# yisol/IDM-VTON

Hardware: NVIDIA H100
Metric: try-on images/sec @768x1024, 30 steps, CFG 2.0 (higher is better)
Workload: dtype fp16

## Files before the change

idm-vton_b200/csrc/attn.cu:

```cuda
#include "common.cuh"
#include "host.h"
#include "wgmma.cuh"

namespace vton {

struct FlashParams {
  __half* out;
  int ld_out;
  int B, H, Nq, N0, N1;
  int D;
  int kv1_off;
  int kv1_count;
  const int* kv1_base;
  int causal;
  float scale_log2;
  int accumulate;
  float out_scale;
};

constexpr int FA_REGION = 128 * 128;
constexpr int FA_STAGES = 2;
constexpr int FA_THREADS = 256;

template <int R>
struct FlashSmem {
  static constexpr int OFF_Q = 0;
  static constexpr int OFF_K = OFF_Q + R * FA_REGION;
  static constexpr int OFF_V = OFF_K + FA_STAGES * R * FA_REGION;
  static constexpr int OFF_BAR = OFF_V + FA_STAGES * R * FA_REGION;
  static constexpr int TOTAL = OFF_BAR + 64 + 1024;
};

__device__ __forceinline__ float fast_exp2(float x) {
  float y;
  asm("ex2.approx.ftz.f32 %0, %1;" : "=f"(y) : "f"(x));
  return y;
}

template <int KS, int R = (KS + 3) / 4, int DN = (KS <= 4 ? 64 : 96)>
__global__ void __launch_bounds__(FA_THREADS, 1)
flash_kernel(const __grid_constant__ CUtensorMap tmQ, const __grid_constant__ CUtensorMap tmK0,
             const __grid_constant__ CUtensorMap tmV0, const __grid_constant__ CUtensorMap tmK1,
             const __grid_constant__ CUtensorMap tmV1, const FlashParams p) {
  using SM = FlashSmem<R>;
  extern __shared__ uint8_t smem_raw[];
  const uint32_t smem_base = (smem_u32(smem_raw) + 1023u) & ~1023u;
  const uint32_t bar_base = smem_base + SM::OFF_BAR;
  const uint32_t q_full = bar_base;
  auto kv_full = [&](int s) { return bar_base + 8u * (1 + s); };
  auto kv_empty = [&](int s) { return bar_base + 8u * (1 + FA_STAGES + s); };

  const int warp = threadIdx.x >> 5;
  const int lane = threadIdx.x & 31;
  const int q_tile = blockIdx.x;
  const int h = blockIdx.y;
  const int b = blockIdx.z;

  if (threadIdx.x == 0) {
    tma_prefetch_desc(&tmQ);
    tma_prefetch_desc(&tmK0);
    tma_prefetch_desc(&tmV0);
    if (p.N1 > 0) {
      tma_prefetch_desc(&tmK1);
      tma_prefetch_desc(&tmV1);
    }
    mbar_init(q_full, 1);
    for (int s = 0; s < FA_STAGES; ++s) {
      mbar_init(kv_full(s), 1);
      mbar_init(kv_empty(s), 2);
    }
    fence_barrier_init();
  }
  pdl_wait();
  __syncthreads();
  pdl_launch_dependents();

  const int tiles0 = (p.N0 + 127) >> 7;
  int idx1 = -1;
  if (p.N1 > 0) {
    idx1 = b - p.kv1_off;
    if (idx1 >= 0) idx1 = idx1 % p.kv1_count + (p.kv1_base ? *p.kv1_base : 0);
  }
  const bool zero_kv = (p.N1 > 0) && (idx1 < 0);
  const int tiles1 = (p.N1 > 0 && idx1 >= 0) ? ((p.N1 + 127) >> 7) : 0;
  const int total = p.causal ? min(tiles0, q_tile + 1) : tiles0 + tiles1;

  auto issue_kv = [&](int j) {
    const int stage = j % FA_STAGES;
    if (j >= FA_STAGES) mbar_wait(kv_empty(stage), ((j / FA_STAGES) - 1) & 1);
    mbar_expect_tx(kv_full(stage), 2 * R * FA_REGION);
#pragma unroll
    for (int r = 0; r < R; ++r) {
      const uint32_t kdst = smem_base + SM::OFF_K + (stage * R + r) * FA_REGION;
      const uint32_t vdst = smem_base + SM::OFF_V + (stage * R + r) * FA_REGION;
      const int col = h * p.D + r * 64;
      if (j < tiles0) {
        tma_load_3d(kdst, &tmK0, kv_full(stage), col, j * 128, b);
        tma_load_3d(vdst, &tmV0, kv_full(stage), col, j * 128, b);
      } else {
        tma_load_3d(kdst, &tmK1, kv_full(stage), col, (j - tiles0) * 128, idx1);
        tma_load_3d(vdst, &tmV1, kv_full(stage), col, (j - tiles0) * 128, idx1);
      }
    }
  };
  if (threadIdx.x == 0) {
    mbar_expect_tx(q_full, R * FA_REGION);
#pragma unroll
    for (int r = 0; r < R; ++r)
      tma_load_3d(smem_base + SM::OFF_Q + r * FA_REGION, &tmQ, q_full, h * p.D + r * 64, q_tile * 128, b);
    for (int j = 0; j < FA_STAGES && j < total; ++j) issue_kv(j);
  }

  const int wg = warp >> 2;
  const int row0 = wg * 64 + ((warp & 3) << 4) + (lane >> 2);
  const int qi0 = q_tile * 128 + row0, qi1 = qi0 + 8;
  const int cq = (lane & 3) * 2;
  const float sl2 = p.scale_log2;
  float m0 = -INFINITY, m1 = -INFINITY, l0 = 0.f, l1 = 0.f;
  float o[DN / 2];
#pragma unroll
  for (int i = 0; i < DN / 2; ++i) o[i] = 0.f;

  mbar_wait(q_full, 0);
  const uint32_t q_src = smem_base + SM::OFF_Q + wg * (64 * 128);
  for (int j = 0; j < total; ++j) {
    const int stage = j % FA_STAGES;
    mbar_wait(kv_full(stage), (j / FA_STAGES) & 1);
    const uint32_t k_src = smem_base + SM::OFF_K + stage * R * FA_REGION;
    const uint32_t v_src = smem_base + SM::OFF_V + stage * R * FA_REGION;
    float s[64];
    wgmma_fence();
#pragma unroll
    for (int k = 0; k < KS; ++k) {
      const uint32_t off = (k >> 2) * FA_REGION + (k & 3) * 32;
      WgmmaF16SS<128, 0>::mma(s, make_gmma_desc_sw128(q_src + off, 0, 1024), make_gmma_desc_sw128(k_src + off, 0, 1024),
                              k > 0 ? 1 : 0);
    }
    wgmma_commit();
    wgmma_wait<0>();
    fence_regs(s);

    const int key0 = (j < tiles0) ? j * 128 : (j - tiles0) * 128;
    const int kv_valid = (j < tiles0) ? min(128, p.N0 - key0) : min(128, p.N1 - key0);
    float mx0 = -INFINITY, mx1 = -INFINITY;
#pragma unroll
    for (int i = 0; i < 16; ++i) {
#pragma unroll
      for (int u = 0; u < 2; ++u) {
        const int col = i * 8 + cq + u;
        bool ok = col < kv_valid;
        const bool ok0 = ok && (!p.causal || key0 + col <= qi0);
        const bool ok1 = ok && (!p.causal || key0 + col <= qi1);
        if (!ok0) s[4 * i + u] = -INFINITY;
        if (!ok1) s[4 * i + 2 + u] = -INFINITY;
        mx0 = fmaxf(mx0, s[4 * i + u]);
        mx1 = fmaxf(mx1, s[4 * i + 2 + u]);
      }
    }
    mx0 = fmaxf(mx0, __shfl_xor_sync(0xffffffffu, mx0, 1));
    mx0 = fmaxf(mx0, __shfl_xor_sync(0xffffffffu, mx0, 2));
    mx1 = fmaxf(mx1, __shfl_xor_sync(0xffffffffu, mx1, 1));
    mx1 = fmaxf(mx1, __shfl_xor_sync(0xffffffffu, mx1, 2));
    const float mn0 = fmaxf(m0, mx0), mn1 = fmaxf(m1, mx1);
    const float alpha0 = fast_exp2((m0 - mn0) * sl2), alpha1 = fast_exp2((m1 - mn1) * sl2);
    const float ms0 = mn0 * sl2, ms1 = mn1 * sl2;
    m0 = mn0;
    m1 = mn1;
    float sum0 = 0.f, sum1 = 0.f;
#pragma unroll
    for (int i = 0; i < 16; ++i) {
#pragma unroll
      for (int u = 0; u < 2; ++u) {
        const float x0 = s[4 * i + u], x1 = s[4 * i + 2 + u];
        const float p0 = x0 == -INFINITY ? 0.f : fast_exp2(x0 * sl2 - ms0);
        const float p1 = x1 == -INFINITY ? 0.f : fast_exp2(x1 * sl2 - ms1);
        s[4 * i + u] = p0;
        s[4 * i + 2 + u] = p1;
        sum0 += p0;
        sum1 += p1;
      }
    }
    l0 = l0 * alpha0 + sum0;
    l1 = l1 * alpha1 + sum1;
#pragma unroll
    for (int i = 0; i < DN / 8; ++i) {
      o[4 * i] *= alpha0;
      o[4 * i + 1] *= alpha0;
      o[4 * i + 2] *= alpha1;
      o[4 * i + 3] *= alpha1;
    }
    uint32_t pa[8][4];
#pragma unroll
    for (int kk = 0; kk < 8; ++kk) {
      pa[kk][0] = pack_h2(s[8 * kk + 0], s[8 * kk + 1]);
      pa[kk][1] = pack_h2(s[8 * kk + 2], s[8 * kk + 3]);
      pa[kk][2] = pack_h2(s[8 * kk + 4], s[8 * kk + 5]);
      pa[kk][3] = pack_h2(s[8 * kk + 6], s[8 * kk + 7]);
    }
    fence_regs(o);
    wgmma_fence();
#pragma unroll
    for (int kk = 0; kk < 8; ++kk)
      WgmmaF16RS<DN>::mma(o, pa[kk], make_gmma_desc_sw128(v_src + kk * 2048, FA_REGION, 1024), 1);
    wgmma_commit();
    wgmma_wait<0>();
    fence_regs(o);
    if ((threadIdx.x & 127) == 0) mbar_arrive(kv_empty(stage));
    if (threadIdx.x == 0 && j + FA_STAGES < total) issue_kv(j + FA_STAGES);
  }

  l0 += __shfl_xor_sync(0xffffffffu, l0, 1);
  l0 += __shfl_xor_sync(0xffffffffu, l0, 2);
  l1 += __shfl_xor_sync(0xffffffffu, l1, 1);
  l1 += __shfl_xor_sync(0xffffffffu, l1, 2);
  if (zero_kv) {
    const float mn0 = fmaxf(m0, 0.f), mn1 = fmaxf(m1, 0.f);
    const float alpha0 = fast_exp2((m0 - mn0) * sl2), alpha1 = fast_exp2((m1 - mn1) * sl2);
    l0 = l0 * alpha0 + static_cast<float>(p.N1) * fast_exp2(-mn0 * sl2);
    l1 = l1 * alpha1 + static_cast<float>(p.N1) * fast_exp2(-mn1 * sl2);
#pragma unroll
    for (int i = 0; i < DN / 8; ++i) {
      o[4 * i] *= alpha0;
      o[4 * i + 1] *= alpha0;
      o[4 * i + 2] *= alpha1;
      o[4 * i + 3] *= alpha1;
    }
  }
  const float inv[2] = {1.f / l0, 1.f / l1};
  const int qi[2] = {qi0, qi1};
#pragma unroll
  for (int hr = 0; hr < 2; ++hr) {
    if (qi[hr] >= p.Nq) continue;
    __half* dst = p.out + (static_cast<long long>(b) * p.Nq + qi[hr]) * p.ld_out + h * p.D;
#pragma unroll
    for (int i = 0; i < DN / 8; ++i) {
      const int col = i * 8 + cq;
      if (col >= p.D) continue;
      float v0 = o[4 * i + 2 * hr] * inv[hr], v1 = o[4 * i + 2 * hr + 1] * inv[hr];
      if (p.accumulate) {
        const float2 a = unpack_h2(*reinterpret_cast<const uint32_t*>(dst + col));
        v0 = a.x + round_h(p.out_scale * round_h(v0));
        v1 = a.y + round_h(p.out_scale * round_h(v1));
      }
      *reinterpret_cast<uint32_t*>(dst + col) = pack_h2(v0, v1);
    }
  }
}

void set_attn_poly(int) {}
void set_attn_qtiles(int) {}
void set_attn_v2(int) {}

static int encode_tokens(CUtensorMap* tm, const void* base, long long ld, int cols, int n, int batch) {
  uint64_t dims[3] = {static_cast<uint64_t>(cols), static_cast<uint64_t>(n), static_cast<uint64_t>(batch)};
  uint64_t strides[2] = {static_cast<uint64_t>(ld) * 2, static_cast<uint64_t>(n) * ld * 2};
  uint32_t box[3] = {64, 128, 1};
  return encode_tmap_f16(tm, base, 3, dims, strides, box);
}

template <int KS>
static int launch_flash(const CUtensorMap& tmQ, const CUtensorMap& tmK0, const CUtensorMap& tmV0, const CUtensorMap& tmK1,
                        const CUtensorMap& tmV1, const FlashParams& p, cudaStream_t stream) {
  constexpr int R = (KS + 3) / 4;
  auto kern = flash_kernel<KS>;
  static bool configured = false;
  if (!configured) {
    VTON_CUDA(cudaFuncSetAttribute(kern, cudaFuncAttributeMaxDynamicSharedMemorySize, FlashSmem<R>::TOTAL));
    configured = true;
  }
  dim3 grid((p.Nq + 127) / 128, p.H, p.B);
  VTON_CUDA(launch_kernel(kern, grid, dim3(FA_THREADS), FlashSmem<R>::TOTAL, stream, tmQ, tmK0, tmV0, tmK1, tmV1, p));
  count_launch();
  return kOk;
}

static int flash(const void* q, long long ldq, const void* k0, const void* v0, long long ldkv0, const void* k1,
                 const void* v1, long long ldkv1, int B1, void* out, long long ldo, FlashParams p, cudaStream_t stream) {
  CUtensorMap tmQ, tmK0, tmV0, tmK1, tmV1;
  const int cols = p.H * p.D;
  if (int e = encode_tokens(&tmQ, q, ldq, cols, p.Nq, p.B)) return e;
  if (int e = encode_tokens(&tmK0, k0, ldkv0, cols, p.N0, p.B)) return e;
  if (int e = encode_tokens(&tmV0, v0, ldkv0, cols, p.N0, p.B)) return e;
  tmK1 = tmK0;
  tmV1 = tmV0;
  if (k1 != nullptr) {
    if (int e = encode_tokens(&tmK1, k1, ldkv1, cols, p.N1, B1)) return e;
    if (int e = encode_tokens(&tmV1, v1, ldkv1, cols, p.N1, B1)) return e;
  }
  p.out = static_cast<__half*>(out);
  p.ld_out = static_cast<int>(ldo);
  switch (p.D / 16) {
    case 1: return launch_flash<1>(tmQ, tmK0, tmV0, tmK1, tmV1, p, stream);
    case 2: return launch_flash<2>(tmQ, tmK0, tmV0, tmK1, tmV1, p, stream);
    case 3: return launch_flash<3>(tmQ, tmK0, tmV0, tmK1, tmV1, p, stream);
    case 4: return launch_flash<4>(tmQ, tmK0, tmV0, tmK1, tmV1, p, stream);
    case 5: return launch_flash<5>(tmQ, tmK0, tmV0, tmK1, tmV1, p, stream);
    case 6: return launch_flash<6>(tmQ, tmK0, tmV0, tmK1, tmV1, p, stream);
  }
  set_last_error("attention: head dim %d unsupported", p.D);
  return kErrUnsupported;
}

int attn_impl(const void* q, long long ldq, const void* k0, const void* v0, long long ldkv0, const void* k1,
              const void* v1, long long ldkv1, void* out, long long ldo, int B, int H, int Nq, int N0, int N1, int B1,
              int kv1_off, int kv1_mod, const void* kv1_base, float scale, int accumulate, cudaStream_t stream) {
  VTON_CHECK_ARG(B > 0 && H > 0 && Nq > 0 && N0 > 0 && N1 >= 0, "attn: bad sizes B=%d H=%d Nq=%d N0=%d N1=%d", B, H, Nq, N0, N1);
  VTON_CHECK_ARG(ldq % 8 == 0 && ldkv0 % 8 == 0 && ldo % 8 == 0, "attn: row strides must be multiples of 8");
  VTON_CHECK_ARG(aligned_to(out, 4), "attn: out must be 4-byte aligned (stored two halves at a time)");
  VTON_CHECK_ARG(B <= 65535 && H <= 65535, "attn: grid too large");
  const bool has1 = N1 > 0 && B1 > 0 && k1 && v1;
  VTON_CHECK_ARG(N1 == 0 || has1 || kv1_off >= B, "attn: segment 1 declared (N1=%d) but no K/V given", N1);
  VTON_CHECK_ARG(!has1 || ldkv1 % 8 == 0, "attn: ldkv1 must be a multiple of 8");
  FlashParams p{};
  p.B = B;
  p.H = H;
  p.Nq = Nq;
  p.N0 = N0;
  p.N1 = N1;
  p.D = 64;
  p.kv1_off = has1 ? kv1_off : (N1 > 0 ? B : 0);
  p.kv1_count = has1 ? (kv1_mod > 0 ? kv1_mod : B1) : 1;
  p.kv1_base = has1 ? static_cast<const int*>(kv1_base) : nullptr;
  p.scale_log2 = scale * 1.4426950408889634f;
  p.accumulate = accumulate;
  p.out_scale = 1.f;
  return flash(q, ldq, k0, v0, ldkv0, has1 ? k1 : nullptr, has1 ? v1 : nullptr, ldkv1, B1, out, ldo, p, stream);
}

int cross_attn_impl(const void* q, long long ldq, const void* kt, const void* vt, long long ldkv_t, int Nt,
                    const void* ki, const void* vi, long long ldkv_i, int Ni, void* out, long long ldo, int B, int H,
                    int Nq, float scale, float ip_scale, cudaStream_t stream) {
  VTON_CHECK_ARG(B > 0 && H > 0 && Nq > 0, "cross_attn: bad sizes B=%d H=%d Nq=%d", B, H, Nq);
  VTON_CHECK_ARG(Nt > 0 && Nt <= 80 && Ni >= 0 && Ni <= 16, "cross_attn: needs 1 <= Nt <= 80 and Ni <= 16 (got %d, %d)", Nt, Ni);
  VTON_CHECK_ARG(q && kt && vt && out && (Ni == 0 || (ki && vi)), "cross_attn: null pointer");
  VTON_CHECK_ARG(ldq % 8 == 0 && ldkv_t % 8 == 0 && ldo % 8 == 0 && (Ni == 0 || ldkv_i % 8 == 0),
                 "cross_attn: row strides must be multiples of 8");
  VTON_CHECK_ARG(aligned_to(out, 4), "cross_attn: out must be 4-byte aligned (stored two halves at a time)");
  VTON_CHECK_ARG(B <= 65535 && H <= 65535, "cross_attn: grid too large");
  FlashParams p{};
  p.B = B;
  p.H = H;
  p.Nq = Nq;
  p.N0 = Nt;
  p.D = 64;
  p.kv1_count = 1;
  p.scale_log2 = scale * 1.4426950408889634f;
  p.out_scale = 1.f;
  if (int e = flash(q, ldq, kt, vt, ldkv_t, nullptr, nullptr, 0, 0, out, ldo, p, stream)) return e;
  if (Ni == 0) return kOk;
  p.N0 = Ni;
  p.accumulate = 1;
  p.out_scale = ip_scale;
  return flash(q, ldq, ki, vi, ldkv_i, nullptr, nullptr, 0, 0, out, ldo, p, stream);
}

int enc_attn_impl(const void* q, long long ldq, const void* k, const void* v, long long ldkv, void* out, long long ldo,
                  int B, int H, int N, int D, float scale, int causal, cudaStream_t stream) {
  VTON_CHECK_ARG(B > 0 && H > 0 && N > 0, "encoder_attention: bad sizes B=%d H=%d N=%d", B, H, N);
  VTON_CHECK_ARG(D >= 16 && D <= 96 && D % 16 == 0, "encoder_attention: head dim %d unsupported (16..96, multiple of 16)", D);
  VTON_CHECK_ARG(ldq % 8 == 0 && ldkv % 8 == 0 && ldo % 8 == 0, "encoder_attention: row strides must be multiples of 8");
  VTON_CHECK_ARG(aligned_to(out, 4), "encoder_attention: out must be 4-byte aligned (stored two halves at a time)");
  VTON_CHECK_ARG(B <= 65535 && H <= 65535, "encoder_attention: grid too large");
  FlashParams p{};
  p.B = B;
  p.H = H;
  p.Nq = N;
  p.N0 = N;
  p.D = D;
  p.kv1_count = 1;
  p.causal = causal ? 1 : 0;
  p.scale_log2 = scale * 1.4426950408889634f;
  p.out_scale = 1.f;
  return flash(q, ldq, k, v, ldkv, nullptr, nullptr, 0, 0, out, ldo, p, stream);
}

}
```

idm-vton_b200/csrc/common.cuh:

```cuda
#pragma once
#include <cuda.h>
#include <cuda_fp16.h>
#include <cuda_runtime.h>
#include <stdint.h>
#include <stdio.h>

namespace vton {


__device__ __forceinline__ uint32_t smem_u32(const void* p) {
  return static_cast<uint32_t>(__cvta_generic_to_shared(p));
}

__device__ __forceinline__ uint64_t globaltimer_ns() {
  uint64_t t;
  asm volatile("mov.u64 %0, %globaltimer;" : "=l"(t));
  return t;
}

__device__ __forceinline__ void mbar_init(uint32_t bar, uint32_t count) {
  asm volatile("mbarrier.init.shared::cta.b64 [%0], %1;" ::"r"(bar), "r"(count) : "memory");
}
__device__ __forceinline__ void fence_barrier_init() {
  asm volatile("fence.mbarrier_init.release.cluster;" ::: "memory");
}
__device__ __forceinline__ void mbar_expect_tx(uint32_t bar, uint32_t bytes) {
  asm volatile("mbarrier.arrive.expect_tx.shared::cta.b64 _, [%0], %1;" ::"r"(bar), "r"(bytes) : "memory");
}
__device__ __forceinline__ void mbar_arrive(uint32_t bar) {
  asm volatile("mbarrier.arrive.shared::cta.b64 _, [%0];" ::"r"(bar) : "memory");
}
__device__ __forceinline__ bool mbar_try_wait(uint32_t bar, uint32_t parity) {
  uint32_t ok;
  asm volatile(
      "{\n\t.reg .pred p;\n\t"
      "mbarrier.try_wait.parity.shared::cta.b64 p, [%1], %2;\n\t"
      "selp.u32 %0, 1, 0, p;\n\t}"
      : "=r"(ok)
      : "r"(bar), "r"(parity)
      : "memory");
  return ok != 0;
}
__device__ __forceinline__ void mbar_wait(uint32_t bar, uint32_t parity) {
  if (mbar_try_wait(bar, parity)) return;
  const uint64_t t0 = globaltimer_ns();
  uint32_t spins = 0;
  while (!mbar_try_wait(bar, parity)) {
    if ((++spins & 0x3ff) == 0 && globaltimer_ns() - t0 > 4000000000ull) __trap();
  }
}

__device__ __forceinline__ void fence_proxy_async_smem() {
  asm volatile("fence.proxy.async.shared::cta;" ::: "memory");
}

__device__ __forceinline__ bool elect_one() {
  uint32_t pred;
  asm volatile(
      "{\n\t.reg .pred p;\n\t"
      "elect.sync _|p, 0xffffffff;\n\t"
      "selp.u32 %0, 1, 0, p;\n\t}"
      : "=r"(pred));
  return pred != 0;
}

__device__ __forceinline__ void tma_prefetch_desc(const CUtensorMap* m) {
  asm volatile("prefetch.tensormap [%0];" ::"l"(reinterpret_cast<uint64_t>(m)) : "memory");
}
__device__ __forceinline__ void tma_load_2d(uint32_t dst, const CUtensorMap* m, uint32_t bar, int c0, int c1) {
  asm volatile(
      "cp.async.bulk.tensor.2d.shared::cluster.global.mbarrier::complete_tx::bytes [%0], [%1, {%3, %4}], [%2];"
      ::"r"(dst), "l"(reinterpret_cast<uint64_t>(m)), "r"(bar), "r"(c0), "r"(c1)
      : "memory");
}
__device__ __forceinline__ void tma_load_3d(uint32_t dst, const CUtensorMap* m, uint32_t bar, int c0, int c1,
                                            int c2) {
  asm volatile(
      "cp.async.bulk.tensor.3d.shared::cluster.global.mbarrier::complete_tx::bytes [%0], [%1, {%3, %4, %5}], [%2];"
      ::"r"(dst), "l"(reinterpret_cast<uint64_t>(m)), "r"(bar), "r"(c0), "r"(c1), "r"(c2)
      : "memory");
}
__device__ __forceinline__ void tma_load_4d(uint32_t dst, const CUtensorMap* m, uint32_t bar, int c0, int c1,
                                            int c2, int c3) {
  asm volatile(
      "cp.async.bulk.tensor.4d.shared::cluster.global.mbarrier::complete_tx::bytes [%0], [%1, {%3, %4, %5, %6}], "
      "[%2];"
      ::"r"(dst), "l"(reinterpret_cast<uint64_t>(m)), "r"(bar), "r"(c0), "r"(c1), "r"(c2), "r"(c3)
      : "memory");
}

__device__ __forceinline__ void pdl_launch_dependents() { asm volatile("griddepcontrol.launch_dependents;" ::: "memory"); }
__device__ __forceinline__ void pdl_wait() { asm volatile("griddepcontrol.wait;" ::: "memory"); }

__device__ __forceinline__ void wgmma_fence() { asm volatile("wgmma.fence.sync.aligned;" ::: "memory"); }
__device__ __forceinline__ void wgmma_commit() { asm volatile("wgmma.commit_group.sync.aligned;" ::: "memory"); }
template <int N>
__device__ __forceinline__ void wgmma_wait() {
  asm volatile("wgmma.wait_group.sync.aligned %0;" ::"n"(N) : "memory");
}
template <int N>
__device__ __forceinline__ void fence_regs(float (&r)[N]) {
#pragma unroll
  for (int i = 0; i < N; ++i) asm volatile("" : "+f"(r[i])::"memory");
}

__device__ __forceinline__ uint64_t make_gmma_desc_sw128(uint32_t saddr, uint32_t lbo_bytes, uint32_t sbo_bytes) {
  uint64_t d = 0;
  d |= static_cast<uint64_t>((saddr & 0x3ffff) >> 4);
  d |= static_cast<uint64_t>((lbo_bytes >> 4) & 0x3fff) << 16;
  d |= static_cast<uint64_t>((sbo_bytes >> 4) & 0x3fff) << 32;
  d |= static_cast<uint64_t>(1) << 62;
  return d;
}

__device__ __forceinline__ void named_bar_sync(uint32_t id, uint32_t nthreads) {
  asm volatile("bar.sync %0, %1;" ::"r"(id), "r"(nthreads) : "memory");
}

__device__ __forceinline__ float h2f(__half h) { return __half2float(h); }
__device__ __forceinline__ __half f2h(float f) { return __float2half_rn(f); }
__device__ __forceinline__ float round_h(float f) { return __half2float(__float2half_rn(f)); }
__device__ __forceinline__ float silu_f(float x) { return x / (1.0f + __expf(-x)); }
__device__ __forceinline__ float gelu_erf_f(float x) { return 0.5f * x * (1.0f + erff(x * 0.70710678118654752f)); }
__device__ __forceinline__ uint32_t pack_h2(float a, float b) {
  __half2 h = __floats2half2_rn(a, b);
  return *reinterpret_cast<uint32_t*>(&h);
}
__device__ __forceinline__ float2 unpack_h2(uint32_t u) {
  __half2 h = *reinterpret_cast<__half2*>(&u);
  return __half22float2(h);
}

}
```

Measured before the change: 0.6061.

## Warp-specialize flash attention with producer warpgroup, pingpong consumers, and fused IP-adapter pass

Restructures the flash attention kernel into a dedicated TMA producer warpgroup plus two consumer warpgroups. Register budgets are rebalanced with setmaxnreg, and the consumers take turns issuing WGMMA through named barriers. For head dim 64 it overlaps the next QK^T with the previous PV matmul, uses three stages when R==1, and skips mask work on full tiles. The IP-adapter attention is also fused into one launch that computes the two softmaxes as separate segments, instead of a second pass that re-reads and accumulates into the output. This adds synchronization complexity and register pressure, and the batch-index rotation adds correctness risk.

```diff
diff --git a/idm-vton_b200/csrc/attn.cu b/idm-vton_b200/csrc/attn.cu
--- a/idm-vton_b200/csrc/attn.cu
+++ b/idm-vton_b200/csrc/attn.cu
@@ -19,15 +19,18 @@
 };
 
 constexpr int FA_REGION = 128 * 128;
-constexpr int FA_STAGES = 2;
-constexpr int FA_THREADS = 256;
+constexpr int FA_THREADS = 384;
+constexpr int FA_PRODUCER_REGS = 40;
+constexpr int FA_CONSUMER_REGS = 232;
+constexpr uint32_t FA_BAR_TURN = 1;
 
 template <int R>
 struct FlashSmem {
+  static constexpr int STAGES = R == 1 ? 3 : 2;
   static constexpr int OFF_Q = 0;
   static constexpr int OFF_K = OFF_Q + R * FA_REGION;
-  static constexpr int OFF_V = OFF_K + FA_STAGES * R * FA_REGION;
-  static constexpr int OFF_BAR = OFF_V + FA_STAGES * R * FA_REGION;
+  static constexpr int OFF_V = OFF_K + STAGES * R * FA_REGION;
+  static constexpr int OFF_BAR = OFF_V + STAGES * R * FA_REGION;
   static constexpr int TOTAL = OFF_BAR + 64 + 1024;
 };
 
@@ -37,26 +40,41 @@
   return y;
 }
 
-template <int KS, int R = (KS + 3) / 4, int DN = (KS <= 4 ? 64 : 96)>
+template <int KS, bool IP = false, int R = (KS + 3) / 4, int DN = (KS <= 4 ? 64 : 96)>
 __global__ void __launch_bounds__(FA_THREADS, 1)
 flash_kernel(const __grid_constant__ CUtensorMap tmQ, const __grid_constant__ CUtensorMap tmK0,
              const __grid_constant__ CUtensorMap tmV0, const __grid_constant__ CUtensorMap tmK1,
              const __grid_constant__ CUtensorMap tmV1, const FlashParams p) {
   using SM = FlashSmem<R>;
+  constexpr int ST = SM::STAGES;
+  constexpr bool OVERLAP = DN == 64 && !IP;
   extern __shared__ uint8_t smem_raw[];
   const uint32_t smem_base = (smem_u32(smem_raw) + 1023u) & ~1023u;
   const uint32_t bar_base = smem_base + SM::OFF_BAR;
   const uint32_t q_full = bar_base;
   auto kv_full = [&](int s) { return bar_base + 8u * (1 + s); };
-  auto kv_empty = [&](int s) { return bar_base + 8u * (1 + FA_STAGES + s); };
+  auto kv_empty = [&](int s) { return bar_base + 8u * (1 + ST + s); };
 
   const int warp = threadIdx.x >> 5;
   const int lane = threadIdx.x & 31;
+  const int wg = threadIdx.x >> 7;
   const int q_tile = blockIdx.x;
   const int h = blockIdx.y;
-  const int b = blockIdx.z;
+  int b = blockIdx.z;
+  if (p.N1 > 0 && p.kv1_off > 0 && p.kv1_off < p.B) {
+    b += p.kv1_off;
+    if (b >= p.B) b -= p.B;
+  }
 
   if (threadIdx.x == 0) {
+    mbar_init(q_full, 1);
+    for (int s = 0; s < ST; ++s) {
+      mbar_init(kv_full(s), 1);
+      mbar_init(kv_empty(s), 2);
+    }
+    fence_barrier_init();
+  }
+  if (threadIdx.x == 256) {
     tma_prefetch_desc(&tmQ);
     tma_prefetch_desc(&tmK0);
     tma_prefetch_desc(&tmV0);
@@ -64,12 +82,6 @@
       tma_prefetch_desc(&tmK1);
       tma_prefetch_desc(&tmV1);
     }
-    mbar_init(q_full, 1);
-    for (int s = 0; s < FA_STAGES; ++s) {
-      mbar_init(kv_full(s), 1);
-      mbar_init(kv_empty(s), 2);
-    }
-    fence_barrier_init();
   }
   pdl_wait();
   __syncthreads();
@@ -85,33 +97,36 @@
   const int tiles1 = (p.N1 > 0 && idx1 >= 0) ? ((p.N1 + 127) >> 7) : 0;
   const int total = p.causal ? min(tiles0, q_tile + 1) : tiles0 + tiles1;
 
-  auto issue_kv = [&](int j) {
-    const int stage = j % FA_STAGES;
-    if (j >= FA_STAGES) mbar_wait(kv_empty(stage), ((j / FA_STAGES) - 1) & 1);
-    mbar_expect_tx(kv_full(stage), 2 * R * FA_REGION);
-#pragma unroll
-    for (int r = 0; r < R; ++r) {
-      const uint32_t kdst = smem_base + SM::OFF_K + (stage * R + r) * FA_REGION;
-      const uint32_t vdst = smem_base + SM::OFF_V + (stage * R + r) * FA_REGION;
-      const int col = h * p.D + r * 64;
-      if (j < tiles0) {
-        tma_load_3d(kdst, &tmK0, kv_full(stage), col, j * 128, b);
-        tma_load_3d(vdst, &tmV0, kv_full(stage), col, j * 128, b);
-      } else {
-        tma_load_3d(kdst, &tmK1, kv_full(stage), col, (j - tiles0) * 128, idx1);
-        tma_load_3d(vdst, &tmV1, kv_full(stage), col, (j - tiles0) * 128, idx1);
-      }
-    }
-  };
-  if (threadIdx.x == 0) {
-    mbar_expect_tx(q_full, R * FA_REGION);
-#pragma unroll
-    for (int r = 0; r < R; ++r)
-      tma_load_3d(smem_base + SM::OFF_Q + r * FA_REGION, &tmQ, q_full, h * p.D + r * 64, q_tile * 128, b);
-    for (int j = 0; j < FA_STAGES && j < total; ++j) issue_kv(j);
-  }
-
-  const int wg = warp >> 2;
+  if (wg == 2) {
+    setmaxnreg_dec<FA_PRODUCER_REGS>();
+    if (threadIdx.x == 256) {
+      mbar_expect_tx(q_full, R * FA_REGION);
+#pragma unroll
+      for (int r = 0; r < R; ++r)
+        tma_load_3d(smem_base + SM::OFF_Q + r * FA_REGION, &tmQ, q_full, h * p.D + r * 64, q_tile * 128, b);
+      for (int j = 0; j < total; ++j) {
+        const int stage = j % ST;
+        if (j >= ST) mbar_wait(kv_empty(stage), ((j / ST) - 1) & 1);
+        mbar_expect_tx(kv_full(stage), 2 * R * FA_REGION);
+#pragma unroll
+        for (int r = 0; r < R; ++r) {
+          const uint32_t kdst = smem_base + SM::OFF_K + (stage * R + r) * FA_REGION;
+          const uint32_t vdst = smem_base + SM::OFF_V + (stage * R + r) * FA_REGION;
+          const int col = h * p.D + r * 64;
+          if (j < tiles0) {
+            tma_load_3d(kdst, &tmK0, kv_full(stage), col, j * 128, b);
+            tma_load_3d(vdst, &tmV0, kv_full(stage), col, j * 128, b);
+          } else {
+            tma_load_3d(kdst, &tmK1, kv_full(stage), col, (j - tiles0) * 128, idx1);
+            tma_load_3d(vdst, &tmV1, kv_full(stage), col, (j - tiles0) * 128, idx1);
+          }
+        }
+      }
+    }
+    return;
+  }
+
+  setmaxnreg_inc<FA_CONSUMER_REGS>();
   const int row0 = wg * 64 + ((warp & 3) << 4) + (lane >> 2);
   const int qi0 = q_tile * 128 + row0, qi1 = qi0 + 8;
   const int cq = (lane & 3) * 2;
@@ -120,15 +135,15 @@
   float o[DN / 2];
 #pragma unroll
   for (int i = 0; i < DN / 2; ++i) o[i] = 0.f;
-
-  mbar_wait(q_full, 0);
+  uint32_t o_seg0[IP ? DN / 4 : 1];
+#pragma unroll
+  for (int i = 0; i < (IP ? DN / 4 : 1); ++i) o_seg0[i] = 0u;
+  float s[64];
+  uint32_t pa[8][4];
+
   const uint32_t q_src = smem_base + SM::OFF_Q + wg * (64 * 128);
-  for (int j = 0; j < total; ++j) {
-    const int stage = j % FA_STAGES;
-    mbar_wait(kv_full(stage), (j / FA_STAGES) & 1);
+  auto issue_s = [&](int stage) {
     const uint32_t k_src = smem_base + SM::OFF_K + stage * R * FA_REGION;
-    const uint32_t v_src = smem_base + SM::OFF_V + stage * R * FA_REGION;
-    float s[64];
     wgmma_fence();
 #pragma unroll
     for (int k = 0; k < KS; ++k) {
@@ -137,24 +152,47 @@
                               k > 0 ? 1 : 0);
     }
     wgmma_commit();
-    wgmma_wait<0>();
-    fence_regs(s);
-
+  };
+  auto issue_pv = [&](int stage) {
+    const uint32_t v_src = smem_base + SM::OFF_V + stage * R * FA_REGION;
+    wgmma_fence();
+#pragma unroll
+    for (int kk = 0; kk < 8; ++kk)
+      WgmmaF16RS<DN>::mma(o, pa[kk], make_gmma_desc_sw128(v_src + kk * 2048, FA_REGION, 1024), 1);
+    wgmma_commit();
+  };
+  auto turn_begin = [&]() { named_bar_sync(FA_BAR_TURN + wg, 256); };
+  auto turn_end = [&](bool last) {
+    if (!(last && wg == 1)) named_bar_arrive(FA_BAR_TURN + (wg ^ 1), 256);
+  };
+  auto softmax = [&](int j, float& alpha0, float& alpha1) {
     const int key0 = (j < tiles0) ? j * 128 : (j - tiles0) * 128;
     const int kv_valid = (j < tiles0) ? min(128, p.N0 - key0) : min(128, p.N1 - key0);
+    const bool masked = p.causal || kv_valid < 128;
     float mx0 = -INFINITY, mx1 = -INFINITY;
-#pragma unroll
-    for (int i = 0; i < 16; ++i) {
-#pragma unroll
-      for (int u = 0; u < 2; ++u) {
-        const int col = i * 8 + cq + u;
-        bool ok = col < kv_valid;
-        const bool ok0 = ok && (!p.causal || key0 + col <= qi0);
-        const bool ok1 = ok && (!p.causal || key0 + col <= qi1);
-        if (!ok0) s[4 * i + u] = -INFINITY;
-        if (!ok1) s[4 * i + 2 + u] = -INFINITY;
-        mx0 = fmaxf(mx0, s[4 * i + u]);
-        mx1 = fmaxf(mx1, s[4 * i + 2 + u]);
+    if (masked) {
+#pragma unroll
+      for (int i = 0; i < 16; ++i) {
+#pragma unroll
+        for (int u = 0; u < 2; ++u) {
+          const int col = i * 8 + cq + u;
+          bool ok = col < kv_valid;
+          const bool ok0 = ok && (!p.causal || key0 + col <= qi0);
+          const bool ok1 = ok && (!p.causal || key0 + col <= qi1);
+          if (!ok0) s[4 * i + u] = -INFINITY;
+          if (!ok1) s[4 * i + 2 + u] = -INFINITY;
+          mx0 = fmaxf(mx0, s[4 * i + u]);
+          mx1 = fmaxf(mx1, s[4 * i + 2 + u]);
+        }
+      }
+    } else {
+#pragma unroll
+      for (int i = 0; i < 16; ++i) {
+#pragma unroll
+        for (int u = 0; u < 2; ++u) {
+          mx0 = fmaxf(mx0, s[4 * i + u]);
+          mx1 = fmaxf(mx1, s[4 * i + 2 + u]);
+        }
       }
     }
     mx0 = fmaxf(mx0, __shfl_xor_sync(0xffffffffu, mx0, 1));
@@ -162,26 +200,54 @@
     mx1 = fmaxf(mx1, __shfl_xor_sync(0xffffffffu, mx1, 1));
     mx1 = fmaxf(mx1, __shfl_xor_sync(0xffffffffu, mx1, 2));
     const float mn0 = fmaxf(m0, mx0), mn1 = fmaxf(m1, mx1);
-    const float alpha0 = fast_exp2((m0 - mn0) * sl2), alpha1 = fast_exp2((m1 - mn1) * sl2);
+    alpha0 = fast_exp2((m0 - mn0) * sl2);
+    alpha1 = fast_exp2((m1 - mn1) * sl2);
     const float ms0 = mn0 * sl2, ms1 = mn1 * sl2;
     m0 = mn0;
     m1 = mn1;
     float sum0 = 0.f, sum1 = 0.f;
-#pragma unroll
-    for (int i = 0; i < 16; ++i) {
-#pragma unroll
-      for (int u = 0; u < 2; ++u) {
-        const float x0 = s[4 * i + u], x1 = s[4 * i + 2 + u];
-        const float p0 = x0 == -INFINITY ? 0.f : fast_exp2(x0 * sl2 - ms0);
-        const float p1 = x1 == -INFINITY ? 0.f : fast_exp2(x1 * sl2 - ms1);
-        s[4 * i + u] = p0;
-        s[4 * i + 2 + u] = p1;
-        sum0 += p0;
-        sum1 += p1;
+    if (masked) {
+#pragma unroll
+      for (int i = 0; i < 16; ++i) {
+#pragma unroll
+        for (int u = 0; u < 2; ++u) {
+          const float x0 = s[4 * i + u], x1 = s[4 * i + 2 + u];
+          const float p0 = x0 == -INFINITY ? 0.f : fast_exp2(x0 * sl2 - ms0);
+          const float p1 = x1 == -INFINITY ? 0.f : fast_exp2(x1 * sl2 - ms1);
+          s[4 * i + u] = p0;
+          s[4 * i + 2 + u] = p1;
+          sum0 += p0;
+          sum1 += p1;
+        }
+      }
+    } else {
+#pragma unroll
+      for (int i = 0; i < 16; ++i) {
+#pragma unroll
+        for (int u = 0; u < 2; ++u) {
+          const float p0 = fast_exp2(s[4 * i + u] * sl2 - ms0);
+          const float p1 = fast_exp2(s[4 * i + 2 + u] * sl2 - ms1);
+          s[4 * i + u] = p0;
+          s[4 * i + 2 + u] = p1;
+          sum0 += p0;
+          sum1 += p1;
+        }
       }
     }
     l0 = l0 * alpha0 + sum0;
     l1 = l1 * alpha1 + sum1;
+  };
+  auto pack_p = [&]() {
+#pragma unroll
+    for (int kk = 0; kk < 8; ++kk) {
+      pa[kk][0] = pack_h2(s[8 * kk + 0], s[8 * kk + 1]);
+      pa[kk][1] = pack_h2(s[8 * kk + 2], s[8 * kk + 3]);
+      pa[kk][2] = pack_h2(s[8 * kk + 4], s[8 * kk + 5]);
+      pa[kk][3] = pack_h2(s[8 * kk + 6], s[8 * kk + 7]);
+    }
+  };
+
+  auto rescale_o = [&](float alpha0, float alpha1) {
 #pragma unroll
     for (int i = 0; i < DN / 8; ++i) {
       o[4 * i] *= alpha0;
@@ -189,24 +255,98 @@
       o[4 * i + 2] *= alpha1;
       o[4 * i + 3] *= alpha1;
     }
-    uint32_t pa[8][4];
-#pragma unroll
-    for (int kk = 0; kk < 8; ++kk) {
-      pa[kk][0] = pack_h2(s[8 * kk + 0], s[8 * kk + 1]);
-      pa[kk][1] = pack_h2(s[8 * kk + 2], s[8 * kk + 3]);
-      pa[kk][2] = pack_h2(s[8 * kk + 4], s[8 * kk + 5]);
-      pa[kk][3] = pack_h2(s[8 * kk + 6], s[8 * kk + 7]);
-    }
-    fence_regs(o);
-    wgmma_fence();
-#pragma unroll
-    for (int kk = 0; kk < 8; ++kk)
-      WgmmaF16RS<DN>::mma(o, pa[kk], make_gmma_desc_sw128(v_src + kk * 2048, FA_REGION, 1024), 1);
-    wgmma_commit();
+  };
+  auto close_segment0 = [&](float ls0, float ls1) {
+    ls0 += __shfl_xor_sync(0xffffffffu, ls0, 1);
+    ls0 += __shfl_xor_sync(0xffffffffu, ls0, 2);
+    ls1 += __shfl_xor_sync(0xffffffffu, ls1, 1);
+    ls1 += __shfl_xor_sync(0xffffffffu, ls1, 2);
+    const float i0 = 1.f / ls0, i1 = 1.f / ls1;
+#pragma unroll
+    for (int i = 0; i < DN / 8; ++i) {
+      if constexpr (IP) {
+        o_seg0[2 * i] = pack_h2(o[4 * i] * i0, o[4 * i + 1] * i0);
+        o_seg0[2 * i + 1] = pack_h2(o[4 * i + 2] * i1, o[4 * i + 3] * i1);
+      }
+      o[4 * i] = o[4 * i + 1] = o[4 * i + 2] = o[4 * i + 3] = 0.f;
+    }
+  };
+
+  if (wg == 1) named_bar_arrive(FA_BAR_TURN, 256);
+  mbar_wait(q_full, 0);
+  if constexpr (OVERLAP) {
+    mbar_wait(kv_full(0), 0);
+    turn_begin();
+    issue_s(0);
+    turn_end(false);
+    wgmma_wait<0>();
+    fence_regs(s);
+    {
+      float a0, a1;
+      softmax(0, a0, a1);
+    }
+    pack_p();
+    for (int j = 1; j < total; ++j) {
+      const int stage = j % ST, prev = (j - 1) % ST;
+      mbar_wait(kv_full(stage), (j / ST) & 1);
+      turn_begin();
+      issue_s(stage);
+      issue_pv(prev);
+      turn_end(false);
+      wgmma_wait<1>();
+      fence_regs(s);
+      const bool seg_start = IP && j == tiles0;
+      float ls0 = l0, ls1 = l1;
+      if (seg_start) {
+        m0 = m1 = -INFINITY;
+        l0 = l1 = 0.f;
+      }
+      float alpha0, alpha1;
+      softmax(j, alpha0, alpha1);
+      wgmma_wait<0>();
+      fence_regs(o);
+      if ((threadIdx.x & 127) == 0) mbar_arrive(kv_empty(prev));
+      if (seg_start)
+        close_segment0(ls0, ls1);
+      else
+        rescale_o(alpha0, alpha1);
+      pack_p();
+    }
+    turn_begin();
+    issue_pv((total - 1) % ST);
+    turn_end(true);
     wgmma_wait<0>();
     fence_regs(o);
-    if ((threadIdx.x & 127) == 0) mbar_arrive(kv_empty(stage));
-    if (threadIdx.x == 0 && j + FA_STAGES < total) issue_kv(j + FA_STAGES);
+  } else {
+    for (int j = 0; j < total; ++j) {
+      const int stage = j % ST;
+      mbar_wait(kv_full(stage), (j / ST) & 1);
+      turn_begin();
+      issue_s(stage);
+      turn_end(false);
+      wgmma_wait<0>();
+      fence_regs(s);
+      const bool seg_start = IP && j == tiles0;
+      float ls0 = l0, ls1 = l1;
+      if (seg_start) {
+        m0 = m1 = -INFINITY;
+        l0 = l1 = 0.f;
+      }
+      float alpha0, alpha1;
+      softmax(j, alpha0, alpha1);
+      if (seg_start)
+        close_segment0(ls0, ls1);
+      else
+        rescale_o(alpha0, alpha1);
+      pack_p();
+      fence_regs(o);
+      turn_begin();
+      issue_pv(stage);
+      turn_end(j == total - 1);
+      wgmma_wait<0>();
+      fence_regs(o);
+      if ((threadIdx.x & 127) == 0) mbar_arrive(kv_empty(stage));
+    }
   }
 
   l0 += __shfl_xor_sync(0xffffffffu, l0, 1);
@@ -228,6 +368,7 @@
   }
   const float inv[2] = {1.f / l0, 1.f / l1};
   const int qi[2] = {qi0, qi1};
+  const bool two_softmax = IP && tiles1 > 0;
 #pragma unroll
   for (int hr = 0; hr < 2; ++hr) {
     if (qi[hr] >= p.Nq) continue;
@@ -237,7 +378,11 @@
       const int col = i * 8 + cq;
       if (col >= p.D) continue;
       float v0 = o[4 * i + 2 * hr] * inv[hr], v1 = o[4 * i + 2 * hr + 1] * inv[hr];
-      if (p.accumulate) {
+      if (two_softmax) {
+        const float2 t = unpack_h2(o_seg0[IP ? 2 * i + hr : 0]);
+        v0 = t.x + round_h(p.out_scale * round_h(v0));
+        v1 = t.y + round_h(p.out_scale * round_h(v1));
+      } else if (p.accumulate) {
         const float2 a = unpack_h2(*reinterpret_cast<const uint32_t*>(dst + col));
         v0 = a.x + round_h(p.out_scale * round_h(v0));
         v1 = a.y + round_h(p.out_scale * round_h(v1));
@@ -258,11 +403,11 @@
   return encode_tmap_f16(tm, base, 3, dims, strides, box);
 }
 
-template <int KS>
+template <int KS, bool IP = false>
 static int launch_flash(const CUtensorMap& tmQ, const CUtensorMap& tmK0, const CUtensorMap& tmV0, const CUtensorMap& tmK1,
                         const CUtensorMap& tmV1, const FlashParams& p, cudaStream_t stream) {
   constexpr int R = (KS + 3) / 4;
-  auto kern = flash_kernel<KS>;
+  auto kern = flash_kernel<KS, IP>;
   static bool configured = false;
   if (!configured) {
     VTON_CUDA(cudaFuncSetAttribute(kern, cudaFuncAttributeMaxDynamicSharedMemorySize, FlashSmem<R>::TOTAL));
@@ -275,7 +420,8 @@
 }
 
 static int flash(const void* q, long long ldq, const void* k0, const void* v0, long long ldkv0, const void* k1,
-                 const void* v1, long long ldkv1, int B1, void* out, long long ldo, FlashParams p, cudaStream_t stream) {
+                 const void* v1, long long ldkv1, int B1, void* out, long long ldo, FlashParams p, cudaStream_t stream,
+                 bool ip = false) {
   CUtensorMap tmQ, tmK0, tmV0, tmK1, tmV1;
   const int cols = p.H * p.D;
   if (int e = encode_tokens(&tmQ, q, ldq, cols, p.Nq, p.B)) return e;
@@ -289,6 +435,7 @@
   }
   p.out = static_cast<__half*>(out);
   p.ld_out = static_cast<int>(ldo);
+  if (ip) return launch_flash<4, true>(tmQ, tmK0, tmV0, tmK1, tmV1, p, stream);
   switch (p.D / 16) {
     case 1: return launch_flash<1>(tmQ, tmK0, tmV0, tmK1, tmV1, p, stream);
     case 2: return launch_flash<2>(tmQ, tmK0, tmV0, tmK1, tmV1, p, stream);
@@ -342,16 +489,13 @@
   p.H = H;
   p.Nq = Nq;
   p.N0 = Nt;
+  p.N1 = Ni;
   p.D = 64;
-  p.kv1_count = 1;
+  p.kv1_count = B;
   p.scale_log2 = scale * 1.4426950408889634f;
-  p.out_scale = 1.f;
-  if (int e = flash(q, ldq, kt, vt, ldkv_t, nullptr, nullptr, 0, 0, out, ldo, p, stream)) return e;
-  if (Ni == 0) return kOk;
-  p.N0 = Ni;
-  p.accumulate = 1;
-  p.out_scale = ip_scale;
-  return flash(q, ldq, ki, vi, ldkv_i, nullptr, nullptr, 0, 0, out, ldo, p, stream);
+  p.out_scale = Ni > 0 ? ip_scale : 1.f;
+  return flash(q, ldq, kt, vt, ldkv_t, Ni > 0 ? ki : nullptr, Ni > 0 ? vi : nullptr, ldkv_i, B, out, ldo, p, stream,
+               Ni > 0);
 }
 
 int enc_attn_impl(const void* q, long long ldq, const void* k, const void* v, long long ldkv, void* out, long long ldo,
diff --git a/idm-vton_b200/csrc/common.cuh b/idm-vton_b200/csrc/common.cuh
--- a/idm-vton_b200/csrc/common.cuh
+++ b/idm-vton_b200/csrc/common.cuh
@@ -116,6 +116,14 @@
 __device__ __forceinline__ void named_bar_sync(uint32_t id, uint32_t nthreads) {
   asm volatile("bar.sync %0, %1;" ::"r"(id), "r"(nthreads) : "memory");
 }
+__device__ __forceinline__ void named_bar_arrive(uint32_t id, uint32_t nthreads) {
+  asm volatile("bar.arrive %0, %1;" ::"r"(id), "r"(nthreads) : "memory");
+}
+
+template <int N>
+__device__ __forceinline__ void setmaxnreg_dec() { asm volatile("setmaxnreg.dec.sync.aligned.u32 %0;" ::"n"(N)); }
+template <int N>
+__device__ __forceinline__ void setmaxnreg_inc() { asm volatile("setmaxnreg.inc.sync.aligned.u32 %0;" ::"n"(N)); }
 
 __device__ __forceinline__ float h2f(__half h) { return __half2float(h); }
 __device__ __forceinline__ __half f2h(float f) { return __float2half_rn(f); }
```

New measurement: 0.6344, median of 6. +4.7%, better.
